# lppllppl920/EndoscopyDepthEstimation-Pytorch

Hardware: AMD Instinct MI355X
Metric: train frame-pairs/sec at 256x320 bs=8 (higher is better)
Workload: dtype f32

## Files before the change

### endoscopydepthestimation-pytorch_amd/csrc/dgrad_newmap_kernels.h

```cpp
#pragma once

#include "dgrad_block_kernels.h"

namespace endo {

template <int NL>
struct NewMapGeom {
    using G = DgradBlockGeom<1, 2, 3, 1, 4>;
    static constexpr int kStage = 12 * G::kCS;
    static constexpr int kW = 9 * 12 * 16;
    static constexpr int kWPre = (kW + kConvThreads - 1) / kConvThreads;
    static constexpr int kConsts = NL * 16 * 4;
    static constexpr size_t kBytes = sizeof(float) * (2 * kStage + NL * kW + kConsts);
    static constexpr int kBlocksPerCu = NL == 1 ? 4 : 3;
    static_assert(kBytes * kBlocksPerCu <= 160 * 1024, "LDS of the resident blocks");
    static_assert(sizeof(double) * 4 * NL * 16 * 2 <= sizeof(float) * kStage, "the final reduction aliases stage 0");
};

template <int NL>
__global__ void __launch_bounds__(kConvThreads, NewMapGeom<NL>::kBlocksPerCu) dgrad_newmap_kernel(const DgradBlockParams p, int tiles_y, int blocks_per_group, int tiles_per_block) {
    using NG = NewMapGeom<NL>;
    using G = typename NG::G;
    constexpr int R = 3;
    extern __shared__ __attribute__((aligned(16))) float smem[];
    float* s_g = smem;
    float* s_w = smem + 2 * NG::kStage;
    float* s_c = s_w + NL * NG::kW;

    const int tid = threadIdx.x;
    const int lane = tid & 63;
    const int wave = __builtin_amdgcn_readfirstlane(tid >> 6);
    const int li = lane & 15;
    const int lk = lane >> 4;
    const int wx = (wave & 1) * 16;
    const int wy = (wave >> 1) * R;

    const int gn = p.group_n > 0 ? p.group_n : p.n;
    const int tps = p.tiles_x * tiles_y;
    const int Q = static_cast<int>(gridDim.x >> 3);
    const bool interleave = (gridDim.x & 7) == 0 && Q > 0 && blocks_per_group % Q == 0;
    int grp, first, t_step, t_last;
    if (interleave) {
        const int lb0 = static_cast<int>(blockIdx.x & 7) * Q;
        grp = lb0 / blocks_per_group;
        const int b0 = lb0 - grp * blocks_per_group;
        first = b0 * tiles_per_block + static_cast<int>(blockIdx.x >> 3);
        t_last = min((b0 + Q) * tiles_per_block, tps * gn);
        t_step = Q;
    } else {
        const int lb = blockIdx.x;
        grp = lb / blocks_per_group;
        first = (lb - grp * blocks_per_group) * tiles_per_block;
        t_last = min(first + tiles_per_block, tps * gn);
        t_step = 1;
    }
    const int ntiles = first < t_last ? (t_last - first + t_step - 1) / t_step : 0;
    if (ntiles <= 0) return;
    const int64_t grp_off = p.group_n > 0 ? grp * p.gs : 0;

    struct Tile { int n, tx, ty, idx; };
    auto place = [&](Tile& t) {
        t.n = t.idx / tps;
        const int rem = t.idx - t.n * tps;
        t.ty = rem / p.tiles_x;
        t.tx = rem - t.ty * p.tiles_x;
    };
    auto advance = [&](Tile& t) { t.idx += t_step; place(t); };
    Tile cur;
    cur.idx = first;
    place(cur);

#pragma unroll
// ... 17 lines not shown
    if (tid < NL * 16) {
        const int l = tid >> 4, j = tid & 15;
        const float* sv = p.saved[0];
        const float* ga = p.gamma[0];
        const float* be = p.beta[0];
        if (NL > 1 && l == 1) { sv = p.saved[1]; ga = p.gamma[1]; be = p.beta[1]; }
        if (NL > 2 && l == 2) { sv = p.saved[2]; ga = p.gamma[2]; be = p.beta[2]; }
        f32x4 c4{0.f, 0.f, 0.f, 0.f};
        if (j < p.count) {
            const float mean = sv[grp_off + 2 * j], rstd = sv[grp_off + 2 * j + 1];
            c4 = f32x4{ga[j] * rstd, be[j], mean, rstd};
        }
        *reinterpret_cast<f32x4*>(s_c + tid * 4) = c4;
    }
    const float wfe = p.vg ? (co_ok ? p.vw[li] : 0.f) : 1.f;

    int u_ry[2], u_rx[2];
#pragma unroll
    for (int k = 0; k < 2; ++k) {
        const int u = lane + 64 * k;
        u_ry[k] = u / (G::kCols / 4);
        u_rx[k] = (u - u_ry[k] * (G::kCols / 4)) * 4;
    }
    const bool second_unit = lane + 64 < G::kUnits;
    const unsigned kOob = 0x80000000u;
    unsigned d_vo[2] = {kOob, kOob};
    const float* d_gn = p.g;
    auto dma_tile = [&](const Tile& t) {
        const int x0 = t.tx * G::kTileX, y0 = t.ty * G::kTileY;
#pragma unroll
        for (int k = 0; k < 2; ++k) {
            const int gy = y0 - 1 + u_ry[k], gx = x0 - G::kLeft + u_rx[k];
            const bool ok = gy >= 0 && gy < p.h && gx >= 0 && gx < p.w;
            d_vo[k] = ok ? 4u * static_cast<unsigned>(gy * p.g_w + gx) : kOob;
        }
        d_gn = p.g + grp_off + static_cast<int64_t>(t.n) * p.g_ns;
    };
    auto issue_chunk = [&](int l, int stage) {
        float* dst = s_g + stage * NG::kStage;
        const __amdgpu_buffer_rsrc_t gr = __builtin_amdgcn_make_buffer_rsrc(const_cast<float*>(d_gn), 0, NL * 12 * p.g_cs * 4, 0x00020000);
#pragma unroll
        for (int i = 0; i < 3; ++i) {
            const int c = wave + 4 * i;
            const unsigned so = 4u * static_cast<unsigned>((l * 12 + c) * p.g_cs);
            __builtin_amdgcn_raw_ptr_buffer_load_lds(gr, (lptr_t)(dst + c * G::kCS), 16, d_vo[0], so, 0, 0);
            if (second_unit) __builtin_amdgcn_raw_ptr_buffer_load_lds(gr, (lptr_t)(dst + c * G::kCS + 256), 16, d_vo[1], so, 0, 0);
        }
    };

    f32x4 xc[R], dc[R], total[R];
    const int lane_x = wx + 4 * lk;
    unsigned lo_r[R];
#pragma unroll
    for (int r = 0; r < R; ++r) lo_r[r] = static_cast<unsigned>(li * p.cs + (wy + r) * p.w + lane_x);
    const unsigned lo_ch = static_cast<unsigned>(li * p.cs);
    int64_t cur_off = 0, po_off = 0, cur_voff = 0;
    unsigned cur_rows = 0, po_rows = 0;
    bool cur_full = false, po_full = false;
    auto begin_tile = [&](const Tile& t) {
        const int x0 = t.tx * G::kTileX, y0 = t.ty * G::kTileY;
        cur_full = y0 + G::kTileY <= p.h && x0 + G::kTileX <= p.w;
        cur_off = grp_off + static_cast<int64_t>(t.n) * p.ns + y0 * p.w + x0;
        cur_voff = grp_off + static_cast<int64_t>(t.n) * p.cs + y0 * p.w + x0;
        const float* xb = p.x + cur_off;
        const float* ob = p.vg ? p.vg + cur_voff : p.out + cur_off;
        if (cur_full) {
            cur_rows = co_ok ? 7u : 0u;
#pragma unroll
            for (int r = 0; r < R; ++r) {
                xc[r] = *reinterpret_cast<const f32x4*>(xb + lo_r[r]);
                dc[r] = *reinterpret_cast<const f32x4*>(ob + (p.vg ? lo_r[r] - lo_ch : lo_r[r]));
            }
        } else {
            unsigned rows = 0;
#pragma unroll
            for (int r = 0; r < R; ++r)
                if (y0 + wy + r < p.h) rows |= 1u << r;
            cur_rows = (co_ok && x0 + lane_x + 3 < p.w) ? rows : 0u;
#pragma unroll
            for (int r = 0; r < R; ++r) {
                xc[r] = f32x4{0.f, 0.f, 0.f, 0.f};
                dc[r] = f32x4{0.f, 0.f, 0.f, 0.f};
                if (cur_rows & (1u << r)) {
                    xc[r] = *reinterpret_cast<const f32x4*>(xb + lo_r[r]);
                    dc[r] = *reinterpret_cast<const f32x4*>(ob + (p.vg ? lo_r[r] - lo_ch : lo_r[r]));
                }
            }
        }
    };

    auto store_results = [&]() {
        float* ob = p.out + po_off;
        if (po_full) {
            if (co_ok) {
#pragma unroll
                for (int r = 0; r < R; ++r) *reinterpret_cast<f32x4*>(ob + lo_r[r]) = dc[r];
            }
        } else {
#pragma unroll
            for (int r = 0; r < R; ++r)
                if (po_rows & (1u << r)) *reinterpret_cast<f32x4*>(ob + lo_r[r]) = dc[r];
        }
    };

    constexpr int kFlushTiles = 8;
    float fs1[NL], fs2[NL];
    double ds1[NL], ds2[NL];
    int tiles_since_flush = 0;
#pragma unroll
    for (int l = 0; l < NL; ++l) { fs1[l] = fs2[l] = 0.f; ds1[l] = ds2[l] = 0.0; }
    dma_tile(cur);
    issue_chunk(0, 0);
    Tile nxt = cur;
    advance(nxt);
    int stage = 0;

    for (int t = 0; t < ntiles; ++t) {
#pragma unroll
        for (int l = 0; l < NL; ++l) {
            asm volatile("s_waitcnt vmcnt(0)" ::: "memory");
            __syncthreads();
            if (l == 0) {
                if (t > 0) {
                    store_results();
                }
                begin_tile(cur);
            }
            if (l + 1 < NL) {
                issue_chunk(l + 1, stage ^ 1);
            } else if (t + 1 < ntiles) {
                dma_tile(nxt);
                issue_chunk(0, stage ^ 1);
            }
            f32x4 acc[R];
#pragma unroll
// ... 16 lines not shown
#pragma unroll
                for (int quad = 0; quad < 3; ++quad) {
                    const int set = quad & 1;
                    if (quad + 1 < 3) load_quad(quad + 1, set ^ 1);
                    __builtin_amdgcn_sched_barrier(0);
#pragma unroll
                    for (int dx = 0; dx < 3; ++dx)
#pragma unroll
                        for (int dy = 0; dy < 3; ++dy)
#pragma unroll
                            for (int r = 0; r < R; ++r)
                                acc[r] = __builtin_amdgcn_mfma_f32_16x16x4f32(av[set][dx][r + dy], bw[set][dy * 3 + dx], acc[r], 0, 0, 0);
                    __builtin_amdgcn_sched_barrier(0);
                }
            }
            {
                const f32x4 c4 = *reinterpret_cast<const f32x4*>(s_c + (l * 16 + li) * 4);
                const float scale = c4[0], beta = c4[1], mean = c4[2], rstd = c4[3];
                float s1 = 0.f, s2 = 0.f;
                auto row = [&](int r) {
#pragma unroll
                    for (int e = 0; e < 4; ++e) {
                        const float xcen = xc[r][e] - mean;
                        const float z = fmaf(xcen, scale, beta);
                        const float dz = z > 0.f ? acc[r][e] : 0.f;
                        s1 += dz;
                        s2 = fmaf(dz, xcen, s2);
                        total[r][e] = l == 0 ? scale * dz : fmaf(scale, dz, total[r][e]);
                    }
                };
// ... 8 lines not shown
                    }
                }
                fs1[l] += s1;
                fs2[l] = fmaf(s2, rstd, fs2[l]);
            }
            if (l == NL - 1) {
#pragma unroll
                for (int r = 0; r < R; ++r)
#pragma unroll
                    for (int e = 0; e < 4; ++e) {
                        float old = dc[r][e] * wfe;
                        asm volatile("" : "+v"(old));
                        dc[r][e] = old + total[r][e];
                    }
                po_off = cur_off;
                po_rows = cur_rows;
                po_full = cur_full;
                cur = nxt;
                advance(nxt);
                if (++tiles_since_flush == kFlushTiles) {
                    tiles_since_flush = 0;
#pragma unroll
                    for (int k = 0; k < NL; ++k) {
                        ds1[k] += static_cast<double>(fs1[k]); ds2[k] += static_cast<double>(fs2[k]);
                        fs1[k] = 0.f; fs2[k] = 0.f;
                    }
                }
            }
            stage ^= 1;
            asm volatile("" : "+s"(stage));
        }
    }
    store_results();

    __syncthreads();
    double* red = reinterpret_cast<double*>(smem);
#pragma unroll
    for (int l = 0; l < NL; ++l) {
        double a = ds1[l] + static_cast<double>(fs1[l]), b = ds2[l] + static_cast<double>(fs2[l]);
        a += __shfl_xor(a, 16, 64); a += __shfl_xor(a, 32, 64);
        b += __shfl_xor(b, 16, 64); b += __shfl_xor(b, 32, 64);
        if (lk == 0) {
            red[((wave * NL + l) * 16 + li) * 2] = a;
            red[((wave * NL + l) * 16 + li) * 2 + 1] = b;
        }
    }
    __syncthreads();
    if (tid < 32 * NL) {
// ... 3 lines not shown
#pragma unroll
            for (int wv = 0; wv < 4; ++wv) t += red[((wv * NL + l) * 16 + j) * 2 + which];
            double* sc = p.scratch[0];
            if (NL > 1 && l == 1) sc = p.scratch[1];
            if (NL > 2 && l == 2) sc = p.scratch[2];
            atomicAdd(sc + bn_slot_offset(p.slot_stride) + grp_off / 2 + 2 * j + which, t);
        }
    }
}

inline bool dgrad_newmap_ok(const DgradBlockParams& p) {
    return p.count <= 16 && p.acc_from == 0 && 36ll * p.g_cs * 4 < (1ll << 31) && (16ll * p.cs + static_cast<int64_t>(p.h) * p.w) * 4 < (1ll << 32);
}

template <int NL>
inline int launch_dgrad_newmap(DgradBlockParams p, hipStream_t stream) {
    using NG = NewMapGeom<NL>;
    using G = typename NG::G;
    p.tiles_x = (p.w + G::kTileX - 1) / G::kTileX;
    const int tiles_y = (p.h + G::kTileY - 1) / G::kTileY;
    const int groups = p.group_n > 0 ? p.n / p.group_n : 1;
    const int tiles_per_group = p.tiles_x * tiles_y * (p.group_n > 0 ? p.group_n : p.n);
    const int resident = device_cu_count() * NG::kBlocksPerCu / groups;
    const int tiles_per_block = (tiles_per_group + resident - 1) / resident;
    int blocks_per_group = (tiles_per_group + tiles_per_block - 1) / tiles_per_block;
    blocks_per_group = (blocks_per_group + 7) / 8 * 8;
    return launch_dyn(dgrad_newmap_kernel<NL>, dim3(groups * blocks_per_group), kConvThreads, NG::kBytes, stream, p, tiles_y, blocks_per_group, tiles_per_block);
}

}
```

### endoscopydepthestimation-pytorch_amd/csrc/net.hip

```cpp
#include <new>
#include <vector>

#include "dgrad_kernels.h"
#include "dgrad_block_kernels.h"
#include "dgrad_newmap_kernels.h"
#include "td_dgrad_kernels.h"
#include "td_fwd_kernels.h"
#include "wgrad_taps_kernels.h"
#include "wgrad1x1_kernels.h"
#include "wgrad_nsplit_kernels.h"
#include "wgrad_x3_kernels.h"
#include "wgrad_f34_kernels.h"
#include "wgrad_subpix_kernels.h"
#include "wino_fwd_kernels.h"
#include "wino4_fwd_kernels.h"
#include "dgrad_wino_kernels.h"
#include "dgrad_wino3_kernels.h"


namespace endo {

int run_dgrad_wino3_nl4(const DgradBlockParams& p, const float* const* u, hipStream_t stream);
bool dgrad_wino3p_applies(const DgradBlockParams& p);
int run_dgrad_wino3p_nl4(const DgradBlockParams& p, const float* const* u, int blocks, double* fw_parts, int* blocks_used, hipStream_t stream);
// ... 119 lines not shown
    int64_t partial_off;
    int64_t wino_off;
    int64_t wino4_off;
    int64_t pq_off;
    int64_t pq_floats;
    int64_t scratch_off;
    int64_t scratch_bytes;
    int64_t slot_stride;
    int64_t wg_scratch_off;
    int64_t tuw_scratch_off;
    int64_t wd_off;
    int64_t gplane_off;
    int64_t bias_parts_off;
    int64_t fw_parts_off;
    int64_t bias_parts_floats;
    int64_t gradws_floats;
    hipStream_t wstream;
    hipEvent_t ev_fork, ev_join;
    int opt[ENDO_OPT_COUNT];
};

namespace endo {


constexpr int kBiasPartChannels = 2048;
constexpr int kBiasPartLaunches = 64;
constexpr int kFwPartBlocks = 512;
struct BiasReduceTable {
    int n;
    struct Entry { const float* parts; float* bias; int count; int nparts; } e[kBiasPartLaunches];
};
struct BiasParts {
    BiasReduceTable table;
    int64_t used;
};

struct BnFin4 {
    const double* scratch[4];
    const float* saved[4];
    const float* gamma[4];
    float* ggamma[4];
// ... 163 lines not shown
        const int b = tile / 3, co = (tile % 3) * 16 + lane16;
        float v = 0.f;
        if (co < cout) {
            const float* src = w + (static_cast<int64_t>(co) * cin + ci) * 9;
            const int ky0 = a == 0 ? (t == 0 ? 0 : 1) : (t == 0 ? 0 : 2), ky1 = a == 0 ? (t == 0 ? 0 : 2) : (t == 0 ? 1 : 2);
            int kx0, kx1;
            if (b == 0) { kx0 = ctap == 0 ? 0 : 1; kx1 = ctap == 0 ? 0 : 2; }
            else { kx0 = ctap == 1 ? 0 : 2; kx1 = ctap == 1 ? 1 : 2; }
            for (int ky = ky0; ky <= ky1; ++ky)
                for (int kx = kx0; kx <= kx1; ++kx) v += src[ky * 3 + kx];
        }
        out[(static_cast<int64_t>(a) * cin + ci) * kPhW + (t * 12 + slot) * 16 + lane16] = v;
    }
}

__global__ void tu_subpix_dgrad_weights_kernel(const float* __restrict__ w, int cout, int cin, float* __restrict__ out) {
    const int pitch = 4 * cin + 16;
    const int total = 4 * cout * 4 * cin;
    for (int i = blockIdx.x * blockDim.x + threadIdx.x; i < total; i += gridDim.x * blockDim.x) {
        const int ci = i % cin;
        const int tap = (i / cin) & 3;
        const int co = (i / (4 * cin)) % cout;
        const int ph = i / (4 * cin * cout);
        const int alpha = ph >> 1, beta = ph & 1, tyi = tap >> 1, txi = tap & 1;
        const int ky0 = alpha == 0 ? (tyi == 0 ? 1 : 0) : (tyi == 0 ? 2 : 0), ky1 = alpha == 0 ? (tyi == 0 ? 2 : 0) : (tyi == 0 ? 2 : 1);
        const int kx0 = beta == 0 ? (txi == 0 ? 1 : 0) : (txi == 0 ? 2 : 0), kx1 = beta == 0 ? (txi == 0 ? 2 : 0) : (txi == 0 ? 2 : 1);
        const float* src = w + (static_cast<int64_t>(co) * cin + ci) * 9;
        float v = 0.f;
        for (int ky = ky0; ky <= ky1; ++ky)
            for (int kx = kx0; kx <= kx1; ++kx) v += src[ky * 3 + kx];
        out[static_cast<int64_t>(ph * cout + co) * pitch + tap * cin + ci] = v;
// ... 142 lines not shown
    bool tu_subpix[kLevels];
};

enum class NewMap { Bf16, Persistent, Vec16, Dword };
enum class BasePass { Block8, Block8Bf16, Wino3, Wino3Persistent, Wino8 };
enum class DenseWgrad { F34, X3, NSplit, Taps, Direct };
enum class TdDgrad { Persistent, Runs128, Dma, Staged };
enum class TuWgrad { Subpix, Taps, Direct };
enum class TuDgrad { Subpix32x8, Subpix16x8, Subpix16x4, Plain };
enum class FirstWgrad { F34Prep, F34, Taps, Direct };
struct BwdPlan {
    struct Block {
        bool fused;
        NewMap newmap[kLayers];
        BasePass base;
        bool wino3_layout;
    } block[kBlocks];
    DenseWgrad wgrad[kDense];
    bool td_wgrad_dma[kLevels];
    TdDgrad td_dgrad[kLevels];
    TuWgrad tu_wgrad[kLevels];
    TuDgrad tu_dgrad[kLevels];
    int overlap;
    bool bf16_wgrad, bf16_dgrad;
    int f34_blocks;
    bool dgrad_weights;
    bool use_virt;
    bool virt_base;
    bool virt_base_w;
    int materialise;
// ... 76 lines not shown
static double conv_flops(const endo_net* net, int level, int cin, int cout, int ks) {
    return 2.0 * net->n * net->groups * net->lv[level].plane * cin * cout * ks * ks;
}

static void default_options(int (&opt)[ENDO_OPT_COUNT]) {
    opt[ENDO_OPT_WINO_FWD] = 5;
    opt[ENDO_OPT_WINO_DGRAD] = 3;
    opt[ENDO_OPT_DGRAD_VEC] = 2;
    opt[ENDO_OPT_WINO_MIN_TILES] = 1024;
    opt[ENDO_OPT_MFMA_BF16] = 0;
    opt[ENDO_OPT_WGRAD_OVERLAP] = 1;
    opt[ENDO_OPT_MFMA_X3] = 0;
    opt[ENDO_OPT_WGRAD_F34] = 1;
    opt[ENDO_OPT_FINAL_VIRTUAL] = 1;
    opt[ENDO_OPT_TD_PERSIST] = 3;
}
static int bf16_mask(const int* opt) { const int v = opt[ENDO_OPT_MFMA_BF16]; return v == 1 ? 7 : (v >> 1); }

struct DenseBlock { int level, ic0, c0; const BnP* bn; const ConvP* cv; bool base_overwrite; };
static DenseBlock dense_block(int b) {
    const Table& tb = table();
    if (b < kLevels) return {b, 48, down_in(b), tb.down_bn[b], tb.down_conv[b], false};
    if (b == kLevels) return {kLevels, 0, 288, tb.bott_bn, tb.bott_conv, true};
    const int i = b - kLevels - 1, l = kLevels - 1 - i;
    return {l, 0, 96 + down_in(l), tb.up_bn[i], tb.up_conv[i], l > 0};
}
static long tile_count(const Ctx& c, int level, int tx, int ty) {
    const auto& lv = c.net->lv[level];
    return static_cast<long>((lv.w + tx - 1) / tx) * ((lv.h + ty - 1) / ty) * c.nt();
}
// ... 346 lines not shown
        const DgradBlockParams base = base_pass_params(c, k);
        bl.fused = dgrad_block_ok(base);
        const long wtiles = static_cast<long>(lv.w / 32) * (lv.h / 8) * c.nt();
        if (pl.bf16_dgrad) bl.base = BasePass::Block8Bf16;
        else if (wino_dgrad != 0 && dgrad_wino_ok(base) && wtiles >= min_tiles)
            bl.base = !((wino_dgrad == 1 || wino_dgrad == 3) && dgrad_wino3_ok(base)) ? BasePass::Wino8
                    : (wino_dgrad == 3 && dgrad_wino3p_applies(base)) ? BasePass::Wino3Persistent : BasePass::Wino3;
        else bl.base = BasePass::Block8;
        bl.wino3_layout = bl.base == BasePass::Wino3 || bl.base == BasePass::Wino3Persistent;
        for (int j = 1; j < kLayers; ++j) {
            const DgradBlockParams p = newmap_params(c, k, j);
            const bool vec = dgrad_block_vec_ok(p);
            bl.newmap[j] = (pl.bf16_dgrad && vec) ? NewMap::Bf16 : (vec && opt[ENDO_OPT_DGRAD_VEC] >= 2 && dgrad_newmap_ok(p)) ? NewMap::Persistent
                         : (vec && opt[ENDO_OPT_DGRAD_VEC] != 0) ? NewMap::Vec16 : NewMap::Dword;
        }
        for (int j = 0; j < kLayers; ++j) {
            const WgradParams p = dense_wgrad_params(c, k, j);
            pl.wgrad[b * kLayers + j] = (f34 && wgrad_f34_ok(p, f34_min_tiles)) ? DenseWgrad::F34 : wgrad_nsplit_ok(p) ? (x3 ? DenseWgrad::X3 : DenseWgrad::NSplit)
                                      : wgrad_taps_ok(p) ? DenseWgrad::Taps : DenseWgrad::Direct;
        }
    }
    for (int l = 0; l < kLevels; ++l) {
        const auto& sv = c.net->lv[l + 1];
        pl.td_wgrad_dma[l] = wgrad1x1_dma_ok(td_wgrad_params(c, l));
        const ConvParams td = td_dgrad_params(c, l);
        const bool persist = (opt[ENDO_OPT_TD_PERSIST] & 1) && !pl.bf16_dgrad;
        pl.td_dgrad[l] = (persist && td_dgrad_ok(td)) ? TdDgrad::Persistent : (persist && sv.w % 4 != 0 && td_dgrad_small_ok(td)) ? TdDgrad::Runs128
                       : sv.w % 4 == 0 ? TdDgrad::Dma : TdDgrad::Staged;
        const ConvP& tu = table().tu_conv[kLevels - 1 - l];
        pl.tu_wgrad[l] = tu_wgrad_subpix_ok(tu_wgrad_params(c, l, true)) ? TuWgrad::Subpix : wgrad_taps_ok(tu_wgrad_params(c, l, false), true) ? TuWgrad::Taps : TuWgrad::Direct;
// ... 51 lines not shown
        fill_in(c, p, c.gbuf(level), level, oc0, cv.cout);
        p.wgt = c.params + cv.w; p.w_cout = cv.cout; p.w_cin = cv.cin;
        fill_out(c, p, c.gbuf(level), level, ic0, cv.cin);
        p.x = c.act(level) + ic0 * lv.plane; p.x_ns = lv.t * lv.plane; p.x_cs = static_cast<int>(lv.plane);
        p.bn_saved = c.saved(bn); p.bn_gamma = c.params + bn.g; p.bn_beta = c.params + bn.b;
        p.bn_scratch = c.scratch(bn); p.bn_slot_stride = c.net->slot_stride;
        p.acc_from = acc_from - ic0;
        ProfScope prof(kProfDgradDense, c.stream, conv_flops(c.net, level, cv.cin, cv.cout, 3), 4.0 * c.nt() * lv.plane * (3.0 * cv.cin + cv.cout));
        rc = launch_dgrad_dense_auto(p, c.stream);
        if (rc) return rc;
    }
    return bn_finalize(c, bn, level, ic0);
}

template <int NL>
static int launch_newmap(NewMap form, const DgradBlockParams& p, hipStream_t stream) {
    switch (form) {
        case NewMap::Bf16: return launch_dgrad_block<NL, 2, 3, 1, 0, 1, 4, 1>(p, stream);
        case NewMap::Persistent: return launch_dgrad_newmap<NL>(p, stream);
        case NewMap::Vec16: return launch_dgrad_block<NL, 2, 3, 1, 0, 1, 4>(p, stream);
        case NewMap::Dword: return launch_dgrad_block<NL, 2, 3>(p, stream);
    }
    return ENDO_E_BADARG;
}

static int dense_block_bwd(const Ctx& c, int b, const FinalVirt* fv = nullptr) {
    const DenseBlock k = dense_block(b);
    const BwdPlan::Block& bl = c.bwd->block[b];
    const int level = k.level, ic0 = k.ic0, c0 = k.c0, new0 = ic0 + c0;
    const auto& lv = c.net->lv[level];
    if (!bl.fused) {
        for (int j = kLayers - 1; j >= 0; --j) {
            const int acc_from = (j == kLayers - 1 && k.base_overwrite) ? new0 : 0;
            int rc = dense_bwd(c, b, j, acc_from < ic0 ? ic0 : acc_from);
            if (rc) return rc;
        }
        return 0;
    }
    BnFin4 pending{};
    int pending_nl = 0;
    F34ReduceBatch red{};
    for (int j = kLayers - 1; j >= 0; --j) {
        int rc = prep_dy(c, level, new0 + kGrowth * j, kGrowth, c.grads + k.cv[j].b, &pending, pending_nl, (fv && j == kLayers - 1) ? fv : nullptr);
        if (rc) return rc;
        const bool defer = c.bwd->overlap == 2;
        if (!defer || j == 0) {
            Ctx cw;
            rc = c.fork_wgrad(cw, level);
            if (rc) return rc;
            for (int jj = defer ? kLayers - 1 : j; jj >= j; --jj) {
                rc = dense_wgrad(cw, b, jj, &red, jj);
                if (rc) return rc;
            }
            if (j == 0 && red.count > 0) {
                ProfScope prof(kProfSmall, cw.stream, 0.0, 0.0);
                rc = launch_wgrad_f34_reduce_batch(red, cw.stream);
                if (rc) return rc;
            }
        }
        if (j > 0) {
            const int nl = kLayers - j;
            BnFin4 a{};
            DgradBlockParams p = newmap_params(c, k, j, &a);
            if (fv) { p.vg = fv->vg; p.vw = fv->vw + ic0 + p.w_ci_off; }
            ProfScope prof(kProfDgradDense, c.stream, 2.0 * c.nt() * lv.plane * kGrowth * kGrowth * 9 * nl,
                           4.0 * c.nt() * lv.plane * (3.0 * kGrowth + kGrowth * nl));
            rc = nl == 1 ? launch_newmap<1>(bl.newmap[j], p, c.stream) : nl == 2 ? launch_newmap<2>(bl.newmap[j], p, c.stream) : launch_newmap<3>(bl.newmap[j], p, c.stream);
            if (rc) return rc;
            pending = a;
            pending_nl = nl;
        }
    }
    {
        DgradBlockParams p = base_pass_params(c, k);
        const bool virt = fv && c.bwd->virt_base;
        if (virt) { p.vg = fv->vg; p.vw = fv->vw + ic0; }
        ProfScope prof(kProfDgradDense, c.stream, 2.0 * c.nt() * lv.plane * c0 * kGrowth * 9 * kLayers,
                       4.0 * c.nt() * lv.plane * (3.0 * c0 + kGrowth * kLayers));
        const float* ub = c.gradws + c.net->wd_off;
        const float* const u[4] = {ub + k.cv[0].ud, ub + k.cv[1].ud, ub + k.cv[2].ud, ub + k.cv[3].ud};
        int rc = 0;
        switch (bl.base) {
            case BasePass::Block8Bf16: rc = launch_dgrad_block8<4, 1>(p, c.stream); break;
// ... 72 lines not shown
        ProfScope prof(kProfWgradOther, cw.stream, conv_flops(c.net, level, cv.cin, cv.cout, 3), 4.0 * c.nt() * lv.plane * (cv.cin / 4.0 + cv.cout));
        rc = form == TuWgrad::Subpix ? launch_tu_wgrad_subpix(p, c.gradws + c.net->wg_scratch_off, cw.stream)
           : form == TuWgrad::Taps ? launch_wgrad_taps<12, IN_UPSAMPLE>(p, cw.stream) : launch_wgrad<3, 1, IN_UPSAMPLE, DY_PLAIN>(p, cw.stream);
        if (rc) return rc;
    }
    ProfScope prof(kProfDgradOther, c.stream, conv_flops(c.net, level, cv.cin, cv.cout, 3), 4.0 * c.nt() * lv.plane * (cv.cout + cv.cin / 4.0));
    const TuDgrad form = c.bwd->tu_dgrad[level];
    if (form == TuDgrad::Plain) {
        ConvParams p{};
        fill_grid(c, p, level);
        fill_in(c, p, c.gbuf(level), level, 0, cv.cout);
        p.wgt = c.params + cv.w; p.w_cout = cv.cout; p.w_cin = cv.cin;
        fill_out(c, p, c.gbuf(src_level), src_level, src_c0, cv.cin);
        return launch_conv_dma_auto<3, 4, 3, IN_PLAIN, EPI_DGRAD_SUMPOOL, 4>(p, c.stream);
    }
    float* wd = c.gradws + c.net->tuw_scratch_off;
    tu_subpix_dgrad_weights_kernel<<<(16 * cv.cout * cv.cin + 255) / 256, 256, 0, c.stream>>>(c.params + cv.w, cv.cout, cv.cin, wd);
    ENDO_LAUNCH_CHECK();
    ConvParams p{};
    fill_grid(c, p, src_level);
    fill_in(c, p, c.gbuf(level), level, 0, 4 * cv.cout);
    p.sub_c = cv.cout;
    p.wgt = wd; p.w_cout = cv.cin; p.w_cin = 4 * cv.cout;
    fill_out(c, p, c.gbuf(src_level), src_level, src_c0, cv.cin);
    if (form == TuDgrad::Subpix32x8) return launch_conv_dma_vec<3, 8, 3, IN_SUBPIX, EPI_FWD, 2, 4, 2, 1, 1>(p, c.stream);
    if (form == TuDgrad::Subpix16x8) return launch_conv_dma_vec<3, 8, 3, IN_SUBPIX, EPI_FWD, 1, 2, 2, 1, 1>(p, c.stream);
    return launch_conv_dma_vec<3, 8, 3, IN_SUBPIX, EPI_FWD, 1, 1, 2, 1, 1>(p, c.stream);
}

static int64_t align_up(int64_t v, int64_t a) { return (v + a - 1) / a * a; }

}

// ... 30 lines not shown
    byte_off += align_up(net->sums_bytes, 256);
    net->partial_off = byte_off / 4;
    byte_off += static_cast<int64_t>(kGrowth) * 163840 * 4;
    net->wino_off = byte_off / 4;
    byte_off += align_up(tb.wino_floats * 4, 256);
    net->wino4_off = byte_off / 4;
    byte_off += align_up(tb.wino4_floats * 4, 256);
    net->tape_floats = byte_off / 4;
    net->pq_off = acts;
    net->pq_floats = 2 * pq;
    net->scratch_off = align_up((acts + net->pq_floats) * 4, 256);
    net->slot_stride = align_up(tb.bn_width_total * 2, 32);
    net->scratch_bytes = net->slot_stride * 8 * kBnSlots;
    net->wg_scratch_off = (net->scratch_off + align_up(net->scratch_bytes, 256)) / 4;
    net->tuw_scratch_off = net->wg_scratch_off + std::max(std::max(kNsScratchFloats, kSpScratchFloats), 4 * kF34ScratchFloats);
    net->wd_off = align_up(net->tuw_scratch_off + 4 * kNew * (4 * kNew + 16), 64);
    net->gplane_off = align_up(net->wd_off + tb.wino_dgrad_floats, 64);
    net->bias_parts_off = net->gplane_off + align_up(static_cast<int64_t>(n) * h * w, 64);
    net->bias_parts_floats = static_cast<int64_t>(kBiasPartChannels) * n * groups * 32;
    {
        int launches = 1, channels = tb.first.cout;
        for (int l = 0; l < kLevels; ++l) {
            for (int j = 0; j < kLayers; ++j) { launches += 2; channels += tb.down_conv[l][j].cout + tb.up_conv[l][j].cout; }
            launches += 2; channels += tb.td_conv[l].cout + tb.tu_conv[l].cout;
        }
        for (int j = 0; j < kLayers; ++j) { ++launches; channels += tb.bott_conv[j].cout; }
        if (launches > kBiasPartLaunches || channels > kBiasPartChannels) { delete net; return ENDO_E_UNSUPPORTED; }
    }
    net->fw_parts_off = net->bias_parts_off + align_up(net->bias_parts_floats, 64);
    net->gradws_floats = net->fw_parts_off + 2 * static_cast<int64_t>(kFwPartBlocks) * 192;
    net->gs = align_up(net->tape_floats > net->gradws_floats ? net->tape_floats : net->gradws_floats, 64);
    *out = net;
    return 0;
}

extern "C" int endo_net_create(endo_net** out, int n, int h, int w) { return endo_net_create_grouped(out, n, h, w, 1); }

extern "C" int endo_net_set_option(endo_net* net, int option_id, int value) {
    if (!net || option_id < 0 || option_id >= ENDO_OPT_COUNT) return ENDO_E_BADARG;
    const int old = net->opt[option_id];
    net->opt[option_id] = value;
    return old;
}

extern "C" int endo_net_get_option(const endo_net* net, int option_id) {
// ... 115 lines not shown
    if (!net->wstream) {
        ENDO_CHECK(hipStreamCreateWithFlags(&net->wstream, hipStreamNonBlocking));
        ENDO_CHECK(hipEventCreateWithFlags(&net->ev_fork, hipEventDisableTiming));
        ENDO_CHECK(hipEventCreateWithFlags(&net->ev_join, hipEventDisableTiming));
    }
    for (int g = 0; g < net->groups; ++g)
        ENDO_CHECK(hipMemsetAsync(gradws + g * net->gs + net->pq_off, 0,
                                  static_cast<size_t>(net->scratch_off + net->scratch_bytes - net->pq_off * 4), c.stream));
    if (plan.dgrad_weights) {
        ProfScope prof(kProfSmall, c.stream, 0.0, 4.0 * 2.0 * tb.wino_dgrad_floats);
        int layout1_blocks = 0;
        for (int b = 0; b < kBlocks; ++b) layout1_blocks |= plan.block[b].wino3_layout ? 1 << b : 0;
        dgrad_wino_weights_kernel<<<(tb.wino_dgrad.start[tb.wino_dgrad.layers] + 255) / 256, 256, 0, c.stream>>>(tb.wino_dgrad, params, gradws + net->wd_off, layout1_blocks);
        ENDO_LAUNCH_CHECK();
    }
    int rc;
    const FinalVirt virt{gradws + net->gplane_off, params + tb.final_.w, grads + tb.final_.w};
    {
        const auto& lv = net->lv[0];
        const int materialise = plan.materialise;
        {
            Ctx cw;
            rc = c.fork_wgrad(cw, 0);
            if (rc) return rc;
            const int c_first = plan.c_first;
            int by = static_cast<int>((lv.plane + 256 * 16 - 1) / (256 * 16));
            by = by < 1 ? 1 : (by > 16 ? 16 : by);
            ProfScope prof(kProfConvFinal, cw.stream, 2.0 * c.nt() * lv.plane * (192 - c_first), 4.0 * c.nt() * lv.plane * (192 - c_first + 2));
            final_bwd_weight_kernel<<<dim3(192 - c_first + 1, by, c.nt()), 256, 0, cw.stream>>>(grad_out, tape + net->pre_off, c.act(0), lv.t * lv.plane,
                                                                         static_cast<int>(lv.plane), 192, net->n, net->gs, grads + tb.final_.w,
// ... 64 lines not shown
```

### endoscopydepthestimation-pytorch_amd/models.py

```python

import ctypes

import torch
from torch import nn

from . import _lib

GROWTH = 12
LAYERS = 4
FIRST = 48
LEVELS = 5


class ConvParams(nn.Module):

    def __init__(self, cin, cout, k):
        super().__init__()
        self.weight = nn.Parameter(torch.empty(cout, cin, k, k))
        self.bias = nn.Parameter(torch.zeros(cout))
        nn.init.kaiming_uniform_(self.weight, a=5 ** 0.5)


class FusedBatchNorm2d(nn.Module):

# ... 218 lines not shown
                p.grad = self._flat_grad[off:off + p.numel()].view(p.shape)

    def _handle(self, n, h, w, groups=1):
        key = (n, h, w, groups)
        if key not in self._handles:
            lib = _lib.load()
            if lib.endo_net_param_floats() != self._flat.numel():
                raise RuntimeError("parameter packing mismatch between Python and libendo_hip.so")
            hnd = ctypes.c_void_p()
            _lib.check(lib.endo_net_create_grouped(ctypes.byref(hnd), n, h, w, groups), "endo_net_create_grouped(%d,%d,%d,%d)" % key)
            for option_id, value in getattr(self, "_kernel_options", {}).items():
                lib.endo_net_set_option(hnd, option_id, value)
            self._handles[key] = (hnd, int(lib.endo_net_tape_floats(hnd)), int(lib.endo_net_gradws_floats(hnd)))
        return self._handles[key]

    _OPTION_DEFAULTS = {0: 5, 1: 3, 2: 2, 3: 1024, 4: 0, 5: 1, 6: 0, 7: 1, 8: 1, 9: 3}

    def set_kernel_option(self, option_id, value):
        option_id, value = int(option_id), int(value)
        if option_id not in self._OPTION_DEFAULTS:
            raise ValueError("unknown kernel option %d" % option_id)
        options = self.__dict__.setdefault("_kernel_options", {})
        old = options.get(option_id, self._OPTION_DEFAULTS[option_id])
        options[option_id] = value
        lib = _lib.load()
        for key, (hnd, _, _) in self._handles.items():
            if key[0] in ("bf16", "fp16"):
                continue
            rc = lib.endo_net_set_option(hnd, option_id, value)
            if rc < 0:
                raise RuntimeError("endo_net_set_option(%d, %d) failed: %d" % (option_id, value, rc))
# ... 334 lines not shown
```

### include/endo_hip.h

```cpp
#ifndef ENDO_HIP_H
#define ENDO_HIP_H

#include <stdint.h>

#ifdef __cplusplus
extern "C" {
#endif

#define ENDO_E_BADARG (-1)
#define ENDO_E_UNSUPPORTED (-2)

#define ENDO_ABI_VERSION 6
int endo_abi_version(void);
const char* endo_error_string(int code);

int endo_depth_scale_fwd(const float* pred, const float* sparse_depth, const float* sparse_mask,
                         float* scaled, float* ratio, double* stats,
                         int n, int hw, float eps, void* stream);
int endo_depth_scale_bwd(const float* grad_scaled, const float* grad_ratio,
                         const float* pred, const float* sparse_depth, const double* stats,
                         float* grad_pred, double* work,
                         int n, int hw, float eps, void* stream);

int endo_flow_from_depth_fwd(const float* depth, const float* mask, const float* t, const float* R,
// ... 66 lines not shown
typedef struct endo_net endo_net;

int endo_net_create(endo_net** out, int n, int h, int w);
int endo_net_create_grouped(endo_net** out, int n, int h, int w, int groups);
int endo_net_groups(const endo_net* net);
#define ENDO_OPT_WINO_FWD 0
#define ENDO_OPT_WINO_DGRAD 1
#define ENDO_OPT_DGRAD_VEC 2
#define ENDO_OPT_WINO_MIN_TILES 3
#define ENDO_OPT_MFMA_BF16 4
#define ENDO_OPT_WGRAD_OVERLAP 5
#define ENDO_OPT_MFMA_X3 6
#define ENDO_OPT_WGRAD_F34 7
#define ENDO_OPT_FINAL_VIRTUAL 8
#define ENDO_OPT_TD_PERSIST 9
#define ENDO_OPT_COUNT 10
int endo_net_set_option(endo_net* net, int option_id, int value);
int endo_net_get_option(const endo_net* net, int option_id);
int64_t endo_net_group_stride(const endo_net* net);
void endo_net_destroy(endo_net* net);
int64_t endo_net_param_floats(void);
int64_t endo_net_bn_floats(void);
int64_t endo_net_tape_floats(const endo_net* net);
int64_t endo_net_gradws_floats(const endo_net* net);
int64_t endo_net_param_offset(int index);
int64_t endo_net_bn_offset(int bn_index, int which );

int endo_net_fwd(endo_net* net, const float* params, float* bn_running, const float* x, float* out,
                 float* tape, int training, void* stream);
int endo_net_bwd(endo_net* net, const float* params, const float* x, const float* tape,
                 const float* grad_out, float* grads, float* gradws, int training, void* stream);
// ... 111 lines not shown
```

Baseline: 514.9.

## Fuse dense-block dy preparation and BN finalize into persistent dgrad kernel

For dense layers 1 and 2, the separate prep_dy pass is folded into the persistent newmap dgrad kernel. The previous layer's dgrad now writes raw gradients to a scratch slot. The next kernel finalizes pending BN sums, applies the p*x+q correction to chunk 0 in LDS, writes the corrected gradient back and accumulates per-block bias partials. Separately, the transposed-subpixel weight transforms for all levels are batched into one launch at the start of the backward pass. This saves launches and a full read/write pass over the gradient, but adds a larger workspace, more LDS traffic and per-channel finalize work in each block.

Measured after the change: 513.6. Within noise of the previous version (-0.3%).

```diff
diff --git a/endoscopydepthestimation-pytorch_amd/csrc/dgrad_newmap_kernels.h b/endoscopydepthestimation-pytorch_amd/csrc/dgrad_newmap_kernels.h
--- a/endoscopydepthestimation-pytorch_amd/csrc/dgrad_newmap_kernels.h
+++ b/endoscopydepthestimation-pytorch_amd/csrc/dgrad_newmap_kernels.h
@@ -12,20 +12,39 @@
     static constexpr int kWPre = (kW + kConvThreads - 1) / kConvThreads;
     static constexpr int kConsts = NL * 16 * 4;
     static constexpr size_t kBytes = sizeof(float) * (2 * kStage + NL * kW + kConsts);
+    static constexpr int kPad = kStage + G::kPlane;
+    static_assert(G::kCS - G::kPlane >= 4 && (kPad % 2) == 0 && (G::kCS % 2) == 0, "room and alignment of the padding words");
     static constexpr int kBlocksPerCu = NL == 1 ? 4 : 3;
     static_assert(kBytes * kBlocksPerCu <= 160 * 1024, "LDS of the resident blocks");
     static_assert(sizeof(double) * 4 * NL * 16 * 2 <= sizeof(float) * kStage, "the final reduction aliases stage 0");
 };
 
-template <int NL>
-__global__ void __launch_bounds__(kConvThreads, NewMapGeom<NL>::kBlocksPerCu) dgrad_newmap_kernel(const DgradBlockParams p, int tiles_y, int blocks_per_group, int tiles_per_block) {
+struct NewMapFused {
+    float* raw_out;
+    const float* raw_in;
+    const float* pq_p;
+    const float* pq_q;
+    const double* fin_scratch[2];
+    const float* fin_saved[2];
+    const float* fin_gamma[2];
+    float* fin_ggamma[2];
+    float* fin_gbeta[2];
+    double count;
+    int training;
+    float* parts;
+};
+
+template <int NL, bool PREP>
+__global__ void __launch_bounds__(kConvThreads, NewMapGeom<NL>::kBlocksPerCu) dgrad_newmap_kernel(const DgradBlockParams p, const NewMapFused fz, int tiles_y, int blocks_per_group, int tiles_per_block) {
     using NG = NewMapGeom<NL>;
     using G = typename NG::G;
     constexpr int R = 3;
+    static_assert(!PREP || (NL >= 2 && NL <= 3), "the pending sums are those of NL - 1 layers");
     extern __shared__ __attribute__((aligned(16))) float smem[];
     float* s_g = smem;
     float* s_w = smem + 2 * NG::kStage;
     float* s_c = s_w + NL * NG::kW;
+    float* s_pad = smem + NG::kPad;
 
     const int tid = threadIdx.x;
     const int lane = tid & 63;
@@ -55,7 +74,10 @@
         t_step = 1;
     }
     const int ntiles = first < t_last ? (t_last - first + t_step - 1) / t_step : 0;
-    if (ntiles <= 0) return;
+    if (ntiles <= 0) {
+        if (PREP && tid < 12) fz.parts[tid * gridDim.x + blockIdx.x] = 0.f;
+        return;
+    }
     const int64_t grp_off = p.group_n > 0 ? grp * p.gs : 0;
 
     struct Tile { int n, tx, ty, idx; };
@@ -103,6 +125,35 @@
         *reinterpret_cast<f32x4*>(s_c + tid * 4) = c4;
     }
     const float wfe = p.vg ? (co_ok ? p.vw[li] : 0.f) : 1.f;
+    if (PREP) {
+        if (tid < 12) {
+            const int c = tid;
+            float pc = fz.pq_p[grp_off + c], qc = fz.pq_q[grp_off + c];
+            double dp = 0.0, dq = 0.0;
+#pragma unroll
+            for (int j = 0; j < NL - 1; ++j) {
+                const double s1 = bn_slot_sum(fz.fin_scratch[j] + grp_off / 2 + 2 * c, p.slot_stride);
+                const double s2 = bn_slot_sum(fz.fin_scratch[j] + grp_off / 2 + 2 * c + 1, p.slot_stride);
+                if (first == 0) {
+                    atomicAdd(fz.fin_ggamma[j] + c, static_cast<float>(s2));
+                    atomicAdd(fz.fin_gbeta[j] + c, static_cast<float>(s1));
+                }
+                if (fz.training) {
+                    const double mean = fz.fin_saved[j][grp_off + 2 * c], rstd = fz.fin_saved[j][grp_off + 2 * c + 1];
+                    const double scale = fz.fin_gamma[j][c] * rstd;
+                    const double k = scale * rstd * s2 / fz.count;
+                    dp += static_cast<double>(static_cast<float>(-k));
+                    dq += static_cast<double>(static_cast<float>(-scale * s1 / fz.count + k * mean));
+                }
+            }
+            pc += static_cast<float>(dp);
+            qc += static_cast<float>(dq);
+            s_pad[c * G::kCS] = pc;
+            s_pad[c * G::kCS + 1] = qc;
+            *reinterpret_cast<double*>(s_pad + c * G::kCS + 2) = 0.0;
+        }
+        __syncthreads();
+    }
 
     int u_ry[2], u_rx[2];
 #pragma unroll
@@ -115,6 +166,7 @@
     const unsigned kOob = 0x80000000u;
     unsigned d_vo[2] = {kOob, kOob};
     const float* d_gn = p.g;
+    int d_n = 0;
     auto dma_tile = [&](const Tile& t) {
         const int x0 = t.tx * G::kTileX, y0 = t.ty * G::kTileY;
 #pragma unroll
@@ -124,10 +176,13 @@
             d_vo[k] = ok ? 4u * static_cast<unsigned>(gy * p.g_w + gx) : kOob;
         }
         d_gn = p.g + grp_off + static_cast<int64_t>(t.n) * p.g_ns;
+        d_n = t.n;
     };
     auto issue_chunk = [&](int l, int stage) {
         float* dst = s_g + stage * NG::kStage;
-        const __amdgpu_buffer_rsrc_t gr = __builtin_amdgcn_make_buffer_rsrc(const_cast<float*>(d_gn), 0, NL * 12 * p.g_cs * 4, 0x00020000);
+        const bool raw = PREP && l == 0;
+        const float* src = raw ? fz.raw_in + grp_off + static_cast<int64_t>(d_n) * (12 * p.g_cs) : d_gn;
+        const __amdgpu_buffer_rsrc_t gr = __builtin_amdgcn_make_buffer_rsrc(const_cast<float*>(src), 0, (raw ? 12 : NL * 12) * p.g_cs * 4, 0x00020000);
 #pragma unroll
         for (int i = 0; i < 3; ++i) {
             const int c = wave + 4 * i;
@@ -136,6 +191,53 @@
             if (second_unit) __builtin_amdgcn_raw_ptr_buffer_load_lds(gr, (lptr_t)(dst + c * G::kCS + 256), 16, d_vo[1], so, 0, 0);
         }
     };
+    f32x4 xr[3][2];
+    float bs[3] = {0.f, 0.f, 0.f};
+    auto load_xj = [&](bool any) {
+        const float* xb = p.x + 12 * p.cs + grp_off + static_cast<int64_t>(d_n) * p.ns;
+#pragma unroll
+        for (int i = 0; i < 3; ++i)
+#pragma unroll
+            for (int k = 0; k < 2; ++k) {
+                xr[i][k] = f32x4{0.f, 0.f, 0.f, 0.f};
+                if (any && (k == 0 || second_unit) && d_vo[k] != kOob) xr[i][k] = *reinterpret_cast<const f32x4*>(xb + (wave + 4 * i) * p.cs + (d_vo[k] >> 2));
+            }
+    };
+    auto flush_bias = [&]() {
+#pragma unroll
+        for (int i = 0; i < 3; ++i) {
+            const double t = wave_sum(static_cast<double>(bs[i]));
+            if (lane == 0) *reinterpret_cast<double*>(s_pad + (wave + 4 * i) * G::kCS + 2) += t;
+            bs[i] = 0.f;
+        }
+    };
+    auto prepare_chunk0 = [&](int stage) {
+        float* sg = s_g + stage * NG::kStage;
+        float* gb = const_cast<float*>(p.g) + grp_off + static_cast<int64_t>(d_n) * p.g_ns;
+#pragma unroll
+        for (int i = 0; i < 3; ++i) {
+            const int c = wave + 4 * i;
+            const float pc = s_pad[c * G::kCS], qc = s_pad[c * G::kCS + 1];
+#pragma unroll
+            for (int k = 0; k < 2; ++k) {
+                if (k == 0 || second_unit) {
+                    float* lp = sg + c * G::kCS + (lane + 64 * k) * 4;
+                    const bool ok = d_vo[k] != kOob;
+                    f32x4 g = *reinterpret_cast<const f32x4*>(lp);
+                    if (ok) {
+#pragma unroll
+                        for (int e = 0; e < 4; ++e) g[e] += fmaf(pc, xr[i][k][e], qc);
+                        *reinterpret_cast<f32x4*>(lp) = g;
+                        if (u_ry[k] >= 1 && u_ry[k] <= G::kTileY && u_rx[k] >= G::kLeft && u_rx[k] < G::kLeft + G::kTileX) {
+                            *reinterpret_cast<f32x4*>(gb + c * p.g_cs + (d_vo[k] >> 2)) = g;
+#pragma unroll
+                            for (int e = 0; e < 4; ++e) bs[i] += g[e];
+                        }
+                    }
+                }
+            }
+        }
+    };
 
     f32x4 xc[R], dc[R], total[R];
     const int lane_x = wx + 4 * lk;
@@ -144,6 +246,7 @@
     for (int r = 0; r < R; ++r) lo_r[r] = static_cast<unsigned>(li * p.cs + (wy + r) * p.w + lane_x);
     const unsigned lo_ch = static_cast<unsigned>(li * p.cs);
     int64_t cur_off = 0, po_off = 0, cur_voff = 0;
+    int64_t cur_roff = 0, po_roff = 0;
     unsigned cur_rows = 0, po_rows = 0;
     bool cur_full = false, po_full = false;
     auto begin_tile = [&](const Tile& t) {
@@ -151,6 +254,7 @@
         cur_full = y0 + G::kTileY <= p.h && x0 + G::kTileX <= p.w;
         cur_off = grp_off + static_cast<int64_t>(t.n) * p.ns + y0 * p.w + x0;
         cur_voff = grp_off + static_cast<int64_t>(t.n) * p.cs + y0 * p.w + x0;
+        cur_roff = grp_off + static_cast<int64_t>(t.n) * (12 * p.cs) + y0 * p.w + x0;
         const float* xb = p.x + cur_off;
         const float* ob = p.vg ? p.vg + cur_voff : p.out + cur_off;
         if (cur_full) {
@@ -179,7 +283,7 @@
     };
 
     auto store_results = [&]() {
-        float* ob = p.out + po_off;
+        float* ob = fz.raw_out ? fz.raw_out + po_roff : p.out + po_off;
         if (po_full) {
             if (co_ok) {
 #pragma unroll
@@ -200,6 +304,7 @@
     for (int l = 0; l < NL; ++l) { fs1[l] = fs2[l] = 0.f; ds1[l] = ds2[l] = 0.0; }
     dma_tile(cur);
     issue_chunk(0, 0);
+    if (PREP) load_xj(true);
     Tile nxt = cur;
     advance(nxt);
     int stage = 0;
@@ -208,6 +313,7 @@
 #pragma unroll
         for (int l = 0; l < NL; ++l) {
             asm volatile("s_waitcnt vmcnt(0)" ::: "memory");
+            if (PREP && l == 0) prepare_chunk0(stage);
             __syncthreads();
             if (l == 0) {
                 if (t > 0) {
@@ -254,6 +360,7 @@
                     __builtin_amdgcn_sched_barrier(0);
                 }
             }
+            if (PREP && l == NL - 1) load_xj(t + 1 < ntiles);
             {
                 const f32x4 c4 = *reinterpret_cast<const f32x4*>(s_c + (l * 16 + li) * 4);
                 const float scale = c4[0], beta = c4[1], mean = c4[2], rstd = c4[3];
@@ -292,6 +399,7 @@
                         dc[r][e] = old + total[r][e];
                     }
                 po_off = cur_off;
+                po_roff = cur_roff;
                 po_rows = cur_rows;
                 po_full = cur_full;
                 cur = nxt;
@@ -303,6 +411,7 @@
                         ds1[k] += static_cast<double>(fs1[k]); ds2[k] += static_cast<double>(fs2[k]);
                         fs1[k] = 0.f; fs2[k] = 0.f;
                     }
+                    if (PREP) flush_bias();
                 }
             }
             stage ^= 1;
@@ -310,6 +419,13 @@
         }
     }
     store_results();
+    if (PREP) {
+        flush_bias();
+        if (lane == 0) {
+#pragma unroll
+            for (int i = 0; i < 3; ++i) fz.parts[(wave + 4 * i) * gridDim.x + blockIdx.x] = static_cast<float>(*reinterpret_cast<const double*>(s_pad + (wave + 4 * i) * G::kCS + 2));
+        }
+    }
 
     __syncthreads();
     double* red = reinterpret_cast<double*>(smem);
@@ -343,18 +459,30 @@
 }
 
 template <int NL>
-inline int launch_dgrad_newmap(DgradBlockParams p, hipStream_t stream) {
+inline int dgrad_newmap_blocks(const DgradBlockParams& p, int* blocks_per_group_out = nullptr, int* tiles_per_block_out = nullptr) {
+    using NG = NewMapGeom<NL>;
+    using G = typename NG::G;
+    const int tiles_x = (p.w + G::kTileX - 1) / G::kTileX, tiles_y = (p.h + G::kTileY - 1) / G::kTileY;
+    const int groups = p.group_n > 0 ? p.n / p.group_n : 1;
+    const int tiles_per_group = tiles_x * tiles_y * (p.group_n > 0 ? p.group_n : p.n);
+    const int resident = device_cu_count() * NG::kBlocksPerCu / groups;
+    const int tiles_per_block = (tiles_per_group + resident - 1) / resident;
+    int blocks_per_group = (tiles_per_group + tiles_per_block - 1) / tiles_per_block;
+    blocks_per_group = (blocks_per_group + 7) / 8 * 8;
+    if (blocks_per_group_out) *blocks_per_group_out = blocks_per_group;
+    if (tiles_per_block_out) *tiles_per_block_out = tiles_per_block;
+    return groups * blocks_per_group;
+}
+
+template <int NL, bool PREP = false>
+inline int launch_dgrad_newmap(DgradBlockParams p, hipStream_t stream, const NewMapFused& fz = NewMapFused{}) {
     using NG = NewMapGeom<NL>;
     using G = typename NG::G;
     p.tiles_x = (p.w + G::kTileX - 1) / G::kTileX;
     const int tiles_y = (p.h + G::kTileY - 1) / G::kTileY;
-    const int groups = p.group_n > 0 ? p.n / p.group_n : 1;
-    const int tiles_per_group = p.tiles_x * tiles_y * (p.group_n > 0 ? p.group_n : p.n);
-    const int resident = device_cu_count() * NG::kBlocksPerCu / groups;
-    const int tiles_per_block = (tiles_per_group + resident - 1) / resident;
-    int blocks_per_group = (tiles_per_group + tiles_per_block - 1) / tiles_per_block;
-    blocks_per_group = (blocks_per_group + 7) / 8 * 8;
-    return launch_dyn(dgrad_newmap_kernel<NL>, dim3(groups * blocks_per_group), kConvThreads, NG::kBytes, stream, p, tiles_y, blocks_per_group, tiles_per_block);
+    int blocks_per_group = 0, tiles_per_block = 0;
+    const int blocks = dgrad_newmap_blocks<NL>(p, &blocks_per_group, &tiles_per_block);
+    return launch_dyn(dgrad_newmap_kernel<NL, PREP>, dim3(blocks), kConvThreads, NG::kBytes, stream, p, fz, tiles_y, blocks_per_group, tiles_per_block);
 }
 
 }
diff --git a/endoscopydepthestimation-pytorch_amd/csrc/net.hip b/endoscopydepthestimation-pytorch_amd/csrc/net.hip
--- a/endoscopydepthestimation-pytorch_amd/csrc/net.hip
+++ b/endoscopydepthestimation-pytorch_amd/csrc/net.hip
@@ -157,6 +157,7 @@
     int64_t bias_parts_off;
     int64_t fw_parts_off;
     int64_t bias_parts_floats;
+    int64_t raw_off;
     int64_t gradws_floats;
     hipStream_t wstream;
     hipEvent_t ev_fork, ev_join;
@@ -168,6 +169,7 @@
 
 constexpr int kBiasPartChannels = 2048;
 constexpr int kBiasPartLaunches = 64;
+constexpr int kNewMapMaxBlocks = 2048;
 constexpr int kFwPartBlocks = 512;
 struct BiasReduceTable {
     int n;
@@ -361,7 +363,15 @@
     }
 }
 
-__global__ void tu_subpix_dgrad_weights_kernel(const float* __restrict__ w, int cout, int cin, float* __restrict__ out) {
+constexpr int64_t kTuwSlotFloats = 4 * kNew * (4 * kNew + 16);
+struct TuSubpixWeightTable { const float* w[kLevels]; };
+__global__ void tu_subpix_dgrad_weights_kernel(const TuSubpixWeightTable tb, int cout, int cin, float* __restrict__ out0) {
+    const float* __restrict__ w = tb.w[0];
+#pragma unroll
+    for (int l = 1; l < kLevels; ++l)
+        if (blockIdx.y == l) w = tb.w[l];
+    if (!w) return;
+    float* __restrict__ out = out0 + blockIdx.y * kTuwSlotFloats;
     const int pitch = 4 * cin + 16;
     const int total = 4 * cout * 4 * cin;
     for (int i = blockIdx.x * blockDim.x + threadIdx.x; i < total; i += gridDim.x * blockDim.x) {
@@ -534,6 +544,7 @@
         bool fused;
         NewMap newmap[kLayers];
         BasePass base;
+        bool prep_fused[kLayers];
         bool wino3_layout;
     } block[kBlocks];
     DenseWgrad wgrad[kDense];
@@ -640,6 +651,7 @@
     opt[ENDO_OPT_WGRAD_F34] = 1;
     opt[ENDO_OPT_FINAL_VIRTUAL] = 1;
     opt[ENDO_OPT_TD_PERSIST] = 3;
+    opt[ENDO_OPT_PREP_FUSED] = 1;
 }
 static int bf16_mask(const int* opt) { const int v = opt[ENDO_OPT_MFMA_BF16]; return v == 1 ? 7 : (v >> 1); }
 
@@ -1016,6 +1028,8 @@
             bl.newmap[j] = (pl.bf16_dgrad && vec) ? NewMap::Bf16 : (vec && opt[ENDO_OPT_DGRAD_VEC] >= 2 && dgrad_newmap_ok(p)) ? NewMap::Persistent
                          : (vec && opt[ENDO_OPT_DGRAD_VEC] != 0) ? NewMap::Vec16 : NewMap::Dword;
         }
+        for (int j = 1; j <= 2; ++j)
+            bl.prep_fused[j] = opt[ENDO_OPT_PREP_FUSED] != 0 && bl.fused && bl.newmap[j] == NewMap::Persistent && bl.newmap[j + 1] == NewMap::Persistent;
         for (int j = 0; j < kLayers; ++j) {
             const WgradParams p = dense_wgrad_params(c, k, j);
             pl.wgrad[b * kLayers + j] = (f34 && wgrad_f34_ok(p, f34_min_tiles)) ? DenseWgrad::F34 : wgrad_nsplit_ok(p) ? (x3 ? DenseWgrad::X3 : DenseWgrad::NSplit)
@@ -1097,10 +1111,13 @@
 }
 
 template <int NL>
-static int launch_newmap(NewMap form, const DgradBlockParams& p, hipStream_t stream) {
+static int launch_newmap(NewMap form, const DgradBlockParams& p, hipStream_t stream, const NewMapFused& fz = NewMapFused{}, bool prep = false) {
+    if (form != NewMap::Persistent && (prep || fz.raw_out)) return ENDO_E_BADARG;
     switch (form) {
         case NewMap::Bf16: return launch_dgrad_block<NL, 2, 3, 1, 0, 1, 4, 1>(p, stream);
-        case NewMap::Persistent: return launch_dgrad_newmap<NL>(p, stream);
+        case NewMap::Persistent:
+            if constexpr (NL >= 2) { if (prep) return launch_dgrad_newmap<NL, true>(p, stream, fz); }
+            return prep ? ENDO_E_BADARG : launch_dgrad_newmap<NL>(p, stream, fz);
         case NewMap::Vec16: return launch_dgrad_block<NL, 2, 3, 1, 0, 1, 4>(p, stream);
         case NewMap::Dword: return launch_dgrad_block<NL, 2, 3>(p, stream);
     }
@@ -1123,33 +1140,70 @@
     BnFin4 pending{};
     int pending_nl = 0;
     F34ReduceBatch red{};
+    const bool defer = c.bwd->overlap == 2;
+    auto fork_wgrads = [&](int j) -> int {
+        if (defer && j != 0) return 0;
+        Ctx cw;
+        int rc = c.fork_wgrad(cw, level);
+        if (rc) return rc;
+        for (int jj = defer ? kLayers - 1 : j; jj >= j; --jj) {
+            rc = dense_wgrad(cw, b, jj, &red, jj);
+            if (rc) return rc;
+        }
+        if (j == 0 && red.count > 0) {
+            ProfScope prof(kProfSmall, cw.stream, 0.0, 0.0);
+            rc = launch_wgrad_f34_reduce_batch(red, cw.stream);
+        }
+        return rc;
+    };
+    auto raw_slot = [&](int j) { return c.gradws + c.net->raw_off + (j & 1) * static_cast<int64_t>(kGrowth) * c.net->n * c.net->lv[0].plane; };
     for (int j = kLayers - 1; j >= 0; --j) {
-        int rc = prep_dy(c, level, new0 + kGrowth * j, kGrowth, c.grads + k.cv[j].b, &pending, pending_nl, (fv && j == kLayers - 1) ? fv : nullptr);
-        if (rc) return rc;
-        const bool defer = c.bwd->overlap == 2;
-        if (!defer || j == 0) {
-            Ctx cw;
-            rc = c.fork_wgrad(cw, level);
+        const bool fused_prep = (j == 1 || j == 2) && bl.prep_fused[j];
+        int rc = 0;
+        if (!fused_prep) {
+            rc = prep_dy(c, level, new0 + kGrowth * j, kGrowth, c.grads + k.cv[j].b, &pending, pending_nl, (fv && j == kLayers - 1) ? fv : nullptr);
             if (rc) return rc;
-            for (int jj = defer ? kLayers - 1 : j; jj >= j; --jj) {
-                rc = dense_wgrad(cw, b, jj, &red, jj);
-                if (rc) return rc;
-            }
-            if (j == 0 && red.count > 0) {
-                ProfScope prof(kProfSmall, cw.stream, 0.0, 0.0);
-                rc = launch_wgrad_f34_reduce_batch(red, cw.stream);
-                if (rc) return rc;
-            }
+            rc = fork_wgrads(j);
+            if (rc) return rc;
         }
         if (j > 0) {
             const int nl = kLayers - j;
             BnFin4 a{};
             DgradBlockParams p = newmap_params(c, k, j, &a);
             if (fv) { p.vg = fv->vg; p.vw = fv->vw + ic0 + p.w_ci_off; }
-            ProfScope prof(kProfDgradDense, c.stream, 2.0 * c.nt() * lv.plane * kGrowth * kGrowth * 9 * nl,
-                           4.0 * c.nt() * lv.plane * (3.0 * kGrowth + kGrowth * nl));
-            rc = nl == 1 ? launch_newmap<1>(bl.newmap[j], p, c.stream) : nl == 2 ? launch_newmap<2>(bl.newmap[j], p, c.stream) : launch_newmap<3>(bl.newmap[j], p, c.stream);
-            if (rc) return rc;
+            NewMapFused fz{};
+            if (j >= 2 && bl.prep_fused[j - 1]) fz.raw_out = raw_slot(j - 1);
+            if (fused_prep) {
+                if (pending_nl != nl - 1 || !c.bias_parts) return ENDO_E_BADARG;
+                const int ch = new0 + kGrowth * j;
+                fz.raw_in = raw_slot(j);
+                fz.pq_p = c.pq_p(level) + ch;
+                fz.pq_q = c.pq_q(level) + ch;
+                for (int l = 0; l < pending_nl; ++l) {
+                    fz.fin_scratch[l] = pending.scratch[l]; fz.fin_saved[l] = pending.saved[l]; fz.fin_gamma[l] = pending.gamma[l];
+                    fz.fin_ggamma[l] = pending.ggamma[l]; fz.fin_gbeta[l] = pending.gbeta[l];
+                }
+                fz.count = static_cast<double>(c.net->n) * lv.h * lv.w;
+                fz.training = c.training;
+                BiasParts& bp = *c.bias_parts;
+                const int blocks = nl == 2 ? dgrad_newmap_blocks<2>(p) : dgrad_newmap_blocks<3>(p);
+                const int64_t need = static_cast<int64_t>(kGrowth) * blocks;
+                if (bp.table.n >= kBiasPartLaunches || bp.used + need > c.net->bias_parts_floats) return ENDO_E_UNSUPPORTED;
+                fz.parts = c.gradws + c.net->bias_parts_off + bp.used;
+                bp.table.e[bp.table.n++] = {fz.parts, c.grads + k.cv[j].b, kGrowth, blocks};
+                bp.used += need;
+            }
+            {
+                ProfScope prof(kProfDgradDense, c.stream, 2.0 * c.nt() * lv.plane * kGrowth * kGrowth * 9 * nl,
+                               4.0 * c.nt() * lv.plane * (3.0 * kGrowth + kGrowth * nl));
+                rc = nl == 1 ? launch_newmap<1>(bl.newmap[j], p, c.stream, fz) : nl == 2 ? launch_newmap<2>(bl.newmap[j], p, c.stream, fz, fused_prep)
+                                                                                         : launch_newmap<3>(bl.newmap[j], p, c.stream, fz, fused_prep);
+                if (rc) return rc;
+            }
+            if (fused_prep) {
+                rc = fork_wgrads(j);
+                if (rc) return rc;
+            }
             pending = a;
             pending_nl = nl;
         }
@@ -1252,9 +1306,7 @@
         fill_out(c, p, c.gbuf(src_level), src_level, src_c0, cv.cin);
         return launch_conv_dma_auto<3, 4, 3, IN_PLAIN, EPI_DGRAD_SUMPOOL, 4>(p, c.stream);
     }
-    float* wd = c.gradws + c.net->tuw_scratch_off;
-    tu_subpix_dgrad_weights_kernel<<<(16 * cv.cout * cv.cin + 255) / 256, 256, 0, c.stream>>>(c.params + cv.w, cv.cout, cv.cin, wd);
-    ENDO_LAUNCH_CHECK();
+    const float* wd = c.gradws + c.net->tuw_scratch_off + level * kTuwSlotFloats;
     ConvParams p{};
     fill_grid(c, p, src_level);
     fill_in(c, p, c.gbuf(level), level, 0, 4 * cv.cout);
@@ -1315,10 +1367,10 @@
     net->scratch_bytes = net->slot_stride * 8 * kBnSlots;
     net->wg_scratch_off = (net->scratch_off + align_up(net->scratch_bytes, 256)) / 4;
     net->tuw_scratch_off = net->wg_scratch_off + std::max(std::max(kNsScratchFloats, kSpScratchFloats), 4 * kF34ScratchFloats);
-    net->wd_off = align_up(net->tuw_scratch_off + 4 * kNew * (4 * kNew + 16), 64);
+    net->wd_off = align_up(net->tuw_scratch_off + kLevels * kTuwSlotFloats, 64);
     net->gplane_off = align_up(net->wd_off + tb.wino_dgrad_floats, 64);
     net->bias_parts_off = net->gplane_off + align_up(static_cast<int64_t>(n) * h * w, 64);
-    net->bias_parts_floats = static_cast<int64_t>(kBiasPartChannels) * n * groups * 32;
+    net->bias_parts_floats = static_cast<int64_t>(kBiasPartChannels) * n * groups * 32 + 2ll * 2 * kLevels * kGrowth * kNewMapMaxBlocks;
     {
         int launches = 1, channels = tb.first.cout;
         for (int l = 0; l < kLevels; ++l) {
@@ -1329,7 +1381,8 @@
         if (launches > kBiasPartLaunches || channels > kBiasPartChannels) { delete net; return ENDO_E_UNSUPPORTED; }
     }
     net->fw_parts_off = net->bias_parts_off + align_up(net->bias_parts_floats, 64);
-    net->gradws_floats = net->fw_parts_off + 2 * static_cast<int64_t>(kFwPartBlocks) * 192;
+    net->raw_off = align_up(net->fw_parts_off + 2 * static_cast<int64_t>(kFwPartBlocks) * 192, 64);
+    net->gradws_floats = net->raw_off + 2 * static_cast<int64_t>(kGrowth) * n * h * w;
     net->gs = align_up(net->tape_floats > net->gradws_floats ? net->tape_floats : net->gradws_floats, 64);
     *out = net;
     return 0;
@@ -1475,6 +1528,17 @@
         dgrad_wino_weights_kernel<<<(tb.wino_dgrad.start[tb.wino_dgrad.layers] + 255) / 256, 256, 0, c.stream>>>(tb.wino_dgrad, params, gradws + net->wd_off, layout1_blocks);
         ENDO_LAUNCH_CHECK();
     }
+    {
+        TuSubpixWeightTable tw{};
+        bool any = false;
+        for (int l = 0; l < kLevels; ++l)
+            if (plan.tu_dgrad[l] != TuDgrad::Plain) { tw.w[l] = params + tb.tu_conv[kLevels - 1 - l].w; any = true; }
+        if (any) {
+            ProfScope prof(kProfSmall, c.stream, 0.0, 4.0 * 2.0 * kLevels * kTuwSlotFloats);
+            tu_subpix_dgrad_weights_kernel<<<dim3((16 * kNew * kNew + 255) / 256, kLevels), 256, 0, c.stream>>>(tw, kNew, kNew, gradws + net->tuw_scratch_off);
+            ENDO_LAUNCH_CHECK();
+        }
+    }
     int rc;
     const FinalVirt virt{gradws + net->gplane_off, params + tb.final_.w, grads + tb.final_.w};
     {
diff --git a/endoscopydepthestimation-pytorch_amd/models.py b/endoscopydepthestimation-pytorch_amd/models.py
--- a/endoscopydepthestimation-pytorch_amd/models.py
+++ b/endoscopydepthestimation-pytorch_amd/models.py
@@ -256,7 +256,7 @@
             self._handles[key] = (hnd, int(lib.endo_net_tape_floats(hnd)), int(lib.endo_net_gradws_floats(hnd)))
         return self._handles[key]
 
-    _OPTION_DEFAULTS = {0: 5, 1: 3, 2: 2, 3: 1024, 4: 0, 5: 1, 6: 0, 7: 1, 8: 1, 9: 3}
+    _OPTION_DEFAULTS = {0: 5, 1: 3, 2: 2, 3: 1024, 4: 0, 5: 1, 6: 0, 7: 1, 8: 1, 9: 3, 10: 1}
 
     def set_kernel_option(self, option_id, value):
         option_id, value = int(option_id), int(value)
diff --git a/include/endo_hip.h b/include/endo_hip.h
--- a/include/endo_hip.h
+++ b/include/endo_hip.h
@@ -104,7 +104,8 @@
 #define ENDO_OPT_WGRAD_F34 7
 #define ENDO_OPT_FINAL_VIRTUAL 8
 #define ENDO_OPT_TD_PERSIST 9
-#define ENDO_OPT_COUNT 10
+#define ENDO_OPT_PREP_FUSED 10
+#define ENDO_OPT_COUNT 11
 int endo_net_set_option(endo_net* net, int option_id, int value);
 int endo_net_get_option(const endo_net* net, int option_id);
 int64_t endo_net_group_stride(const endo_net* net);
```
